# eth-ait/GauSTAR

Measured on AMD Instinct MI355X. Metric: views/sec fwd+bwd @1920x1080, 500k Gaussians; HBM GB/s vs roofline, higher is better.
Workload: dtype f32

## Files before the change

gaustar_amd/csrc/gsr_sort.h:

```cpp
#pragma once
#include "gsr_internal.h"

namespace gsr {

template <int D>
__device__ __forceinline__ uint32_t lane_xor_u32(uint32_t v)
{
    if constexpr (D == 1) return (uint32_t)__builtin_amdgcn_mov_dpp((int)v, 0xB1, 0xf, 0xf, true);
    else if constexpr (D == 2) return (uint32_t)__builtin_amdgcn_mov_dpp((int)v, 0x4E, 0xf, 0xf, true);
    else if constexpr (D == 4) return (uint32_t)__builtin_amdgcn_ds_swizzle((int)v, 0x101F);
    else if constexpr (D == 8) return (uint32_t)__builtin_amdgcn_ds_swizzle((int)v, 0x201F);
    else if constexpr (D == 16) return (uint32_t)__builtin_amdgcn_ds_swizzle((int)v, 0x401F);
    else return (uint32_t)__shfl_xor((int)v, 32, 64);
}
template <int E, int D>
__device__ __forceinline__ void cross_lane_stage(uint64_t (&v)[E], uint32_t e0, uint32_t k, int lane)
{
    const bool lower = (lane & D) == 0;
#pragma unroll
    for (int r = 0; r < E; r++) {
        const uint64_t pv = ((uint64_t)lane_xor_u32<D>((uint32_t)(v[r] >> 32)) << 32) | lane_xor_u32<D>((uint32_t)v[r]);
        const bool asc = ((e0 + r) & k) == 0;
        const bool take_min = lower == asc;
        const bool gt = v[r] > pv;
        v[r] = (gt == take_min) ? pv : v[r];
    }
}

template <int E>
__device__ __forceinline__ void sort_tile_in_registers(uint64_t* __restrict__ s, const uint64_t* __restrict__ gk,
                                                       uint32_t* __restrict__ out, uint32_t n, uint32_t np2)
{
    const int tid = threadIdx.x, lane = tid & 63;
    const uint32_t e0 = (uint32_t)tid * E;
    if (e0 >= np2) {
        if (np2 > 64u * E) {
            for (uint32_t k = 128u * E; k <= np2; k <<= 1)
                for (uint32_t j = k >> 1; j >= 64u * E; j >>= 1) { __syncthreads(); __syncthreads(); }
        }
        return;
    }
    uint64_t v[E];
#pragma unroll
    for (int r = 0; r < E; r++) v[r] = e0 + r < n ? gk[e0 + r] : ~0ull;
    for (uint32_t k = 2; k <= np2; k <<= 1) {
        for (uint32_t j = k >> 1; j > 0; j >>= 1) {
            if (j < (uint32_t)E) {
#pragma unroll
                for (int jj = 1; jj < E; jj <<= 1) {
                    if ((uint32_t)jj != j) continue;
#pragma unroll
                    for (int r = 0; r < E; r++) {
                        if (r & jj) continue;
                        const bool asc = ((e0 + r) & k) == 0;
                        const uint64_t a = v[r], b = v[r | jj];
                        const bool gt = a > b;
                        const uint64_t mn = gt ? b : a, mx = gt ? a : b;
                        v[r] = asc ? mn : mx;
                        v[r | jj] = asc ? mx : mn;
                    }
                }
            } else if (j < 64u * E) {
                switch (j / E) {
                    case 1: cross_lane_stage<E, 1>(v, e0, k, lane); break;
                    case 2: cross_lane_stage<E, 2>(v, e0, k, lane); break;
                    case 4: cross_lane_stage<E, 4>(v, e0, k, lane); break;
                    case 8: cross_lane_stage<E, 8>(v, e0, k, lane); break;
                    case 16: cross_lane_stage<E, 16>(v, e0, k, lane); break;
                    default: cross_lane_stage<E, 32>(v, e0, k, lane); break;
                }
            } else {
#pragma unroll
                for (int r = 0; r < E; r++) s[e0 + r] = v[r];
                __syncthreads();
                const bool lower = (e0 & j) == 0;
#pragma unroll
                for (int r = 0; r < E; r++) {
                    const uint64_t pv = s[(e0 + r) ^ j];
                    const bool asc = ((e0 + r) & k) == 0;
                    const bool take_min = lower == asc;
                    const bool gt = v[r] > pv;
                    v[r] = (gt == take_min) ? pv : v[r];
                }
                __syncthreads();
            }
        }
    }
#pragma unroll
    for (int r = 0; r < E; r++)
        if (e0 + r < n) out[e0 + r] = (uint32_t)v[r];
}

constexpr uint32_t SORT_SMALL_CAP = 2048;

template <uint32_t K, uint32_t J>
__device__ __forceinline__ void run64_stages(uint64_t (&v)[1], int lane)
{
    cross_lane_stage<1, (int)J>(v, (uint32_t)lane, K, lane);
    if constexpr (J > 1) run64_stages<K, J / 2>(v, lane);
    else if constexpr (K < 64) run64_stages<K * 2, K>(v, lane);
}

struct NoStamp { __device__ __forceinline__ void operator()() const {} };
template <int E, class STAMP = NoStamp>
__device__ __forceinline__ const uint64_t* sort_tile_merge(uint64_t* __restrict__ s, const uint64_t* __restrict__ gk,
                                                uint32_t* __restrict__ out, uint32_t n, uint64_t* __restrict__ out_keys = nullptr,
                                                STAMP stamp = STAMP())
{
    const uint32_t tid = threadIdx.x, lane = tid & 63u, wave = tid >> 6;
    uint64_t* A = s;
    uint64_t* B = s + SORT_SMALL_CAP;
    const uint32_t n_runs = (n + 63u) >> 6;
    uint64_t kv[E];
#pragma unroll
    for (int q = 0; q < E; q++) {
        const uint32_t i = (wave + 4u * (uint32_t)q) * 64u + lane;
        kv[q] = i < n ? gk[i] : ~0ull;
    }
#pragma unroll
    for (int q = 0; q < E; q++) {
        const uint32_t r = wave + 4u * (uint32_t)q;
        if (r < n_runs) {
            uint64_t v[1] = {kv[q]};
            run64_stages<2, 1>(v, (int)lane);
            A[r * 64u + lane] = v[0];
        }
    }
    __syncthreads();
    stamp();
    const uint32_t o0 = tid * (uint32_t)E;
    for (uint32_t len = 64u; len < n; len <<= 1) {
        uint64_t res[E];
        if (o0 < n) {
            const uint32_t base = o0 & ~(2u * len - 1u);
            const uint32_t la = min(len, n - base);
            const uint32_t lb = base + len < n ? min(len, n - base - len) : 0u;
            const uint64_t* a = A + base;
            const uint64_t* b = A + base + len;
            const uint32_t d = o0 - base;
            uint32_t lo = d > lb ? d - lb : 0u, hi = min(d, la);
#ifndef GSR_SORT_KARY
#define GSR_SORT_KARY 4
#endif
#if GSR_SORT_KARY == 4
            while (lo < hi) {
                const uint32_t span = hi - lo;
                const uint32_t m1 = lo + (span >> 2), m2 = lo + (span >> 1), m3 = lo + ((3u * span) >> 2);
                const uint64_t a1 = a[m1], b1 = b[d - 1u - m1], a2 = a[m2], b2 = b[d - 1u - m2], a3 = a[m3], b3 = b[d - 1u - m3];
                const bool p1 = a1 < b1, p2 = a2 < b2, p3 = a3 < b3;
                if (!p1) hi = m1;
                else if (!p2) { lo = m1 + 1u; hi = m2; }
                else if (!p3) { lo = m2 + 1u; hi = m3; }
                else lo = m3 + 1u;
            }
#else
            while (lo < hi) {
                const uint32_t mid = (lo + hi) >> 1;
                if (a[mid] < b[d - 1u - mid]) lo = mid + 1u; else hi = mid;
            }
#endif
            const uint32_t ai = lo, bi = d - lo;
            uint64_t ka[E], kb[E];
#pragma unroll
            for (int e = 0; e < E; e++) {
                ka[e] = ai + (uint32_t)e < la ? a[ai + e] : ~0ull;
                kb[e] = bi + (uint32_t)e < lb ? b[bi + e] : ~0ull;
            }
#pragma unroll
            for (int e = 0; e < E; e++) res[e] = ka[e] < kb[E - 1 - e] ? ka[e] : kb[E - 1 - e];
#pragma unroll
            for (int j = E / 2; j > 0; j >>= 1) {
#pragma unroll
                for (int e = 0; e < E; e++) {
                    if ((e & j) == 0) {
                        const uint64_t x = res[e], y = res[e | j];
                        const bool gt = x > y;
                        res[e] = gt ? y : x;
                        res[e | j] = gt ? x : y;
                    }
                }
            }
#pragma unroll
            for (int e = 0; e < E; e++)
                if (o0 + (uint32_t)e < n) B[o0 + e] = res[e];
        }
        __syncthreads();
        stamp();
        uint64_t* t = A; A = B; B = t;
    }
    if (out_keys != nullptr) { for (uint32_t i = tid; i < n; i += 256u) out_keys[i] = A[i]; }
    else { for (uint32_t i = tid; i < n; i += 256u) out[i] = (uint32_t)A[i]; }
    return A;
}

template <class STAMP = NoStamp>
__device__ __forceinline__ const uint64_t* sort_small_tile(uint64_t* __restrict__ s, const uint64_t* __restrict__ gk,
                                                           uint32_t* __restrict__ out, uint32_t n, STAMP stamp = STAMP())
{
    if (n == 1) {
        if (threadIdx.x == 0) out[0] = (uint32_t)gk[0];
        return nullptr;
    }
    if (n <= 512u) return sort_tile_merge<2>(s, gk, out, n, nullptr, stamp);
    if (n <= 1024u) return sort_tile_merge<4>(s, gk, out, n, nullptr, stamp);
    return sort_tile_merge<8>(s, gk, out, n, nullptr, stamp);
}

}
```

Measured before the change: 4922.

## Sort 256-key runs in registers and use DPP/permlane swaps for lane exchange

The per-tile sort now builds initial sorted runs of 64*SORT_RUN_E keys (256 by default) entirely in registers with a bitonic network, instead of 64-key runs. Two LDS merge-path passes and their barriers are skipped. Cross-lane exchanges for distances 4 to 32 switch from ds_swizzle/shfl to DPP moves and the gfx950 permlane16/32 swap builtins, which keeps the exchanges on the VALU path. In exchange it raises register pressure (more keys per thread) and adds more compare-exchange work per thread. A partial-tile fallback sorts runs one at a time.

```diff
diff --git a/gaustar_amd/csrc/gsr_sort.h b/gaustar_amd/csrc/gsr_sort.h
--- a/gaustar_amd/csrc/gsr_sort.h
+++ b/gaustar_amd/csrc/gsr_sort.h
@@ -13,13 +13,36 @@
     else if constexpr (D == 16) return (uint32_t)__builtin_amdgcn_ds_swizzle((int)v, 0x401F);
     else return (uint32_t)__shfl_xor((int)v, 32, 64);
 }
+typedef uint32_t sort_u32x2 __attribute__((ext_vector_type(2)));
+template <int D>
+__device__ __forceinline__ uint32_t lane_xor_valu(uint32_t v, uint32_t lane)
+{
+    if constexpr (D == 1 || D == 2) return lane_xor_u32<D>(v);
+    else if constexpr (D == 4) {
+        const int m = __builtin_amdgcn_mov_dpp((int)v, 0x141, 0xf, 0xf, true);
+        return (uint32_t)__builtin_amdgcn_mov_dpp(m, 0x1B, 0xf, 0xf, true);
+    } else if constexpr (D == 8) return (uint32_t)__builtin_amdgcn_mov_dpp((int)v, 0x128, 0xf, 0xf, true);
+    else if constexpr (D == 16) {
+        const sort_u32x2 r = __builtin_amdgcn_permlane16_swap(v, v, false, false);
+        return (lane & 16u) ? r[0] : r[1];
+    } else {
+        static_assert(D == 32, "lane exchange of 1 .. 32");
+        const sort_u32x2 r = __builtin_amdgcn_permlane32_swap(v, v, false, false);
+        return (lane & 32u) ? r[0] : r[1];
+    }
+}
+template <int D>
+__device__ __forceinline__ uint64_t lane_xor_key(uint64_t v, uint32_t lane)
+{
+    return ((uint64_t)lane_xor_valu<D>((uint32_t)(v >> 32), lane) << 32) | lane_xor_valu<D>((uint32_t)v, lane);
+}
 template <int E, int D>
 __device__ __forceinline__ void cross_lane_stage(uint64_t (&v)[E], uint32_t e0, uint32_t k, int lane)
 {
     const bool lower = (lane & D) == 0;
 #pragma unroll
     for (int r = 0; r < E; r++) {
-        const uint64_t pv = ((uint64_t)lane_xor_u32<D>((uint32_t)(v[r] >> 32)) << 32) | lane_xor_u32<D>((uint32_t)v[r]);
+        const uint64_t pv = lane_xor_key<D>(v[r], (uint32_t)lane);
         const bool asc = ((e0 + r) & k) == 0;
         const bool take_min = lower == asc;
         const bool gt = v[r] > pv;
@@ -92,13 +115,51 @@
 }
 
 constexpr uint32_t SORT_SMALL_CAP = 2048;
-
-template <uint32_t K, uint32_t J>
-__device__ __forceinline__ void run64_stages(uint64_t (&v)[1], int lane)
-{
-    cross_lane_stage<1, (int)J>(v, (uint32_t)lane, K, lane);
-    if constexpr (J > 1) run64_stages<K, J / 2>(v, lane);
-    else if constexpr (K < 64) run64_stages<K * 2, K>(v, lane);
+#ifndef GSR_SORT_RUN_E
+#define GSR_SORT_RUN_E 4
+#endif
+constexpr int SORT_RUN_E = GSR_SORT_RUN_E;
+constexpr uint32_t SORT_RUN = 64u * SORT_RUN_E;
+static_assert(SORT_RUN_E == 1 || SORT_RUN_E == 2 || SORT_RUN_E == 4, "register runs of 64 / 128 / 256 keys");
+
+template <int R, int S, uint32_t K, uint32_t J>
+__device__ __forceinline__ void run_stages(uint64_t (&v)[R * S], uint32_t lane)
+{
+    const auto desc = [&](int r) { return K < (uint32_t)R ? (((uint32_t)r & K) != 0u) : (((lane * (uint32_t)R) & K) != 0u); };
+    if constexpr (J < (uint32_t)R) {
+#pragma unroll
+        for (int s = 0; s < S; s++) {
+#pragma unroll
+            for (int r = 0; r < R; r++) {
+                if (r & (int)J) continue;
+                const uint64_t a = v[s * R + r], b = v[s * R + (r | (int)J)];
+                const bool gt = a > b;
+                const uint64_t mn = gt ? b : a, mx = gt ? a : b;
+                v[s * R + r] = desc(r) ? mx : mn;
+                v[s * R + (r | (int)J)] = desc(r) ? mn : mx;
+            }
+        }
+    } else {
+        constexpr int D = (int)(J / (uint32_t)R);
+        const bool lower = (lane & (uint32_t)D) == 0u;
+#pragma unroll
+        for (int s = 0; s < S; s++) {
+#pragma unroll
+            for (int r = 0; r < R; r++) {
+                const uint64_t pv = lane_xor_key<D>(v[s * R + r], lane);
+                const bool take_min = lower != desc(r);
+                const bool gt = v[s * R + r] > pv;
+                v[s * R + r] = (gt == take_min) ? pv : v[s * R + r];
+            }
+        }
+    }
+    if constexpr (J > 1) run_stages<R, S, K, J / 2>(v, lane);
+    else if constexpr (K < 64u * R) run_stages<R, S, K * 2, K>(v, lane);
+}
+template <int S>
+__device__ __forceinline__ void sort_runs(uint64_t (&v)[SORT_RUN_E * S], uint32_t lane)
+{
+    run_stages<SORT_RUN_E, S, 2, 1>(v, lane);
 }
 
 struct NoStamp { __device__ __forceinline__ void operator()() const {} };
@@ -107,29 +168,46 @@
                                                 uint32_t* __restrict__ out, uint32_t n, uint64_t* __restrict__ out_keys = nullptr,
                                                 STAMP stamp = STAMP())
 {
+    constexpr int R = SORT_RUN_E;
+    constexpr int S = (256 * E + 4 * (int)SORT_RUN - 1) / (4 * (int)SORT_RUN);
     const uint32_t tid = threadIdx.x, lane = tid & 63u, wave = tid >> 6;
     uint64_t* A = s;
     uint64_t* B = s + SORT_SMALL_CAP;
-    const uint32_t n_runs = (n + 63u) >> 6;
-    uint64_t kv[E];
-#pragma unroll
-    for (int q = 0; q < E; q++) {
-        const uint32_t i = (wave + 4u * (uint32_t)q) * 64u + lane;
-        kv[q] = i < n ? gk[i] : ~0ull;
-    }
-#pragma unroll
-    for (int q = 0; q < E; q++) {
-        const uint32_t r = wave + 4u * (uint32_t)q;
-        if (r < n_runs) {
-            uint64_t v[1] = {kv[q]};
-            run64_stages<2, 1>(v, (int)lane);
-            A[r * 64u + lane] = v[0];
+    const uint32_t n_runs = (n + SORT_RUN - 1u) / SORT_RUN;
+    uint64_t kv[R * S];
+#pragma unroll
+    for (int q = 0; q < S; q++) {
+#pragma unroll
+        for (int r = 0; r < R; r++) {
+            const uint32_t i = (wave + 4u * (uint32_t)q) * SORT_RUN + lane * (uint32_t)R + (uint32_t)r;
+            kv[q * R + r] = i < n ? gk[i] : ~0ull;
+        }
+    }
+    const auto put = [&](uint32_t q, const uint64_t* v) {
+        uint64_t* d = A + (wave + 4u * q) * SORT_RUN + lane * (uint32_t)R;
+#pragma unroll
+        for (int r = 0; r < R; r++) d[r] = v[r];
+    };
+    if (wave + 4u * (uint32_t)(S - 1) < n_runs) {
+        sort_runs<S>(kv, lane);
+#pragma unroll
+        for (int q = 0; q < S; q++) put((uint32_t)q, kv + q * R);
+    } else {
+#pragma unroll
+        for (int q = 0; q < S - 1; q++) {
+            if (wave + 4u * (uint32_t)q < n_runs) {
+                uint64_t v[R];
+#pragma unroll
+                for (int r = 0; r < R; r++) v[r] = kv[q * R + r];
+                sort_runs<1>(v, lane);
+                put((uint32_t)q, v);
+            }
         }
     }
     __syncthreads();
     stamp();
     const uint32_t o0 = tid * (uint32_t)E;
-    for (uint32_t len = 64u; len < n; len <<= 1) {
+    for (uint32_t len = SORT_RUN; len < n; len <<= 1) {
         uint64_t res[E];
         if (o0 < n) {
             const uint32_t base = o0 & ~(2u * len - 1u);
```

After: 4944, median of 6. Within noise of the previous version (+0.5%).
